# SciLifeLab/TIDDIT

Hardware: AMD Instinct MI355X
Metric: cov bins/sec, 30x WGS synthetic (signals clustered/sec: see 'dbscan') (higher is better)
Workload: dtype int64; 1 GPU; BASELINE configs[1]: coverage histogram, 24 contigs x 125000000 bp (3.00 Gb), 30x 150-bp sorted stream, 500-bp bins, q>=20 filter; contigs split over the 1 rank(s); reads=600000000, bins=6000000

## Files before the change

tiddit_amd/csrc/tdt_coverage.hip:

```cpp
extern const char *const tdt_variant_coverage;
const char *const tdt_variant_coverage = ""
#ifdef COV_MIN_WAVES
    " COV_MIN_WAVES"
#endif
#ifdef COV_MIN_WAVES1
    " COV_MIN_WAVES1"
#endif
#ifdef COV_MIN_WAVES1_4
    " COV_MIN_WAVES1_4"
#endif
#ifdef COV_MIN_WAVES4
    " COV_MIN_WAVES4"
#endif
#ifdef COV_RPL
    " COV_RPL"
#endif
#ifdef COV_RPL1
    " COV_RPL1"
#endif
#ifdef COV_SPARES1
    " COV_SPARES1"
#endif
#ifdef COV_WIN
    " COV_WIN"
#endif
#ifdef COV_WIN1
    " COV_WIN1"
#endif
    ;

#include "tdt_common.h"

#include <algorithm>
#include <thread>

#define COV_THREADS 256
#ifndef COV_RPL
#define COV_RPL 8
#endif
#ifndef COV_RPL1
#define COV_RPL1 4
#endif
#define COV_READS_PER_BLOCK 16384
#ifndef COV_WIN
#define COV_WIN 2048
#endif
#define COV_LUT_LDS_MAX 1024
#define COV_PUSH_CHUNK (4u << 20)
#define COV_STATUS_BYTES (128 + COV_KEPT_SLOTS * 128)
#define COV_KEPT_SLOTS 512

struct CovItem {
    const int32_t *start;
    const int32_t *end;
    const uint8_t *mapq;
    const uint16_t *flag;
    const unsigned long long *packed;
    unsigned long long n;
    unsigned long long *acc;
    const unsigned long long *lut_end;
    int nbins;
    int aligned;
    unsigned first_block;
    unsigned binned;
};

struct CovParams {
    CovItem it;
    const CovItem *items;
    int n_items;
    int bin_size;
    unsigned magic;
    int shift;
    int min_q;
    int margin;
    unsigned xmax, m15;
    int k15;
    const unsigned long long *lut_main;
    unsigned long long one;
    int *status;
    unsigned long long *kept;
};

__device__ __forceinline__ int cov_div(int x, unsigned magic, int shift) {
    return shift < 0 ? x : (int)(__umulhi((unsigned)x, magic) >> shift);
}

#define DPP_WAVE_SHL1 0x130
#define DPP_WAVE_SHR1 0x138

template <int CTRL>
__device__ __forceinline__ unsigned long long dpp_u64(unsigned long long v) {
    const unsigned lo = __builtin_amdgcn_update_dpp(0u, (unsigned)v, CTRL, 0xf, 0xf, true);
    const unsigned hi = __builtin_amdgcn_update_dpp(0u, (unsigned)(v >> 32), CTRL, 0xf, 0xf, true);
    return ((unsigned long long)hi << 32) | lo;
}

#define COV_DPP_SHR1 "row_shr:1 row_mask:0xf bank_mask:0xf bound_ctrl:0"
#define COV_DPP_SHR2 "row_shr:2 row_mask:0xf bank_mask:0xf bound_ctrl:0"
#define COV_DPP_SHR4 "row_shr:4 row_mask:0xf bank_mask:0xf bound_ctrl:0"
#define COV_DPP_SHR8 "row_shr:8 row_mask:0xf bank_mask:0xf bound_ctrl:0"
#define COV_DPP_BC15 "row_bcast:15 row_mask:0xa bank_mask:0xf"
#define COV_DPP_BC31 "row_bcast:31 row_mask:0xc bank_mask:0xf"
#define COV_SCAN_ALL(STEP) \
    "s_nop 1\n\t" STEP(COV_DPP_SHR1) STEP(COV_DPP_SHR2) STEP(COV_DPP_SHR4) STEP(COV_DPP_SHR8) STEP(COV_DPP_BC15) STEP(COV_DPP_BC31) "s_nop 1"
#define COV_SCAN_STEP(CTRL)                                                                     \
    "v_add_co_u32_dpp %0, vcc, %0, %0 " CTRL "\n\t"                                             \
    "v_addc_co_u32_dpp %1, vcc, %1, %1, vcc " CTRL "\n\t"                                       \
    "v_add_co_u32_dpp %2, vcc, %2, %2 " CTRL "\n\t"                                             \
    "v_addc_co_u32_dpp %3, vcc, %3, %3, vcc " CTRL "\n\t"                                       \
    "v_add_co_u32_dpp %4, vcc, %4, %4 " CTRL "\n\t"                                             \
    "v_addc_co_u32_dpp %5, vcc, %5, %5, vcc " CTRL "\n\t"

__device__ __forceinline__ void wave_scan3_u64(unsigned long long &a0, unsigned long long &a1, unsigned long long &a2) {
    unsigned l0 = (unsigned)a0, h0 = (unsigned)(a0 >> 32), l1 = (unsigned)a1, h1 = (unsigned)(a1 >> 32),
             l2 = (unsigned)a2, h2 = (unsigned)(a2 >> 32);
    asm volatile(COV_SCAN_ALL(COV_SCAN_STEP) : "+v"(l0), "+v"(h0), "+v"(l1), "+v"(h1), "+v"(l2), "+v"(h2)::"vcc", "memory");
    a0 = ((unsigned long long)h0 << 32) | l0;
    a1 = ((unsigned long long)h1 << 32) | l1;
    a2 = ((unsigned long long)h2 << 32) | l2;
}

__device__ __forceinline__ unsigned long long cov_mask_lt(unsigned a, unsigned lim_uniform) {
    unsigned long long m;
    asm("v_cmp_gt_u32_e64 %0, %1, %2" : "=s"(m) : "s"(lim_uniform), "v"(a));
    return m;
}
__device__ __forceinline__ unsigned long long cov_mask_eq0(unsigned a) {
    unsigned long long m;
    asm("v_cmp_eq_u32_e64 %0, 0, %1" : "=s"(m) : "v"(a));
    return m;
}
__device__ __forceinline__ unsigned long long cov_mask_ne0(unsigned a) {
    unsigned long long m;
    asm("v_cmp_ne_u32_e64 %0, 0, %1" : "=s"(m) : "v"(a));
// ... 65 lines not shown
}

template <int RPL>
struct CovTile {
    int s[RPL], e[RPL];
    unsigned mq[RPL / 4];
    unsigned fl[RPL / 2];
};

template <int RPL>
__device__ __forceinline__ CovTile<RPL> cov_load(const CovItem &P, unsigned long long idx, unsigned long long r1) {
    CovTile<RPL> t;
    if (P.aligned && idx + RPL <= r1) {
#pragma unroll
        for (int k = 0; k < RPL / 4; k++) {
            const int4 s4 = *reinterpret_cast<const int4 *>(P.start + idx + 4 * k);
            const int4 e4 = *reinterpret_cast<const int4 *>(P.end + idx + 4 * k);
            t.s[4 * k] = s4.x; t.s[4 * k + 1] = s4.y; t.s[4 * k + 2] = s4.z; t.s[4 * k + 3] = s4.w;
            t.e[4 * k] = e4.x; t.e[4 * k + 1] = e4.y; t.e[4 * k + 2] = e4.z; t.e[4 * k + 3] = e4.w;
        }
        if (RPL == 8) {
            const uint2 m2 = *reinterpret_cast<const uint2 *>(P.mapq + idx);
            const uint4 f4 = *reinterpret_cast<const uint4 *>(P.flag + idx);
            t.mq[0] = m2.x; t.mq[RPL / 4 - 1] = m2.y;
            t.fl[0] = f4.x; t.fl[1] = f4.y; t.fl[RPL / 2 - 2] = f4.z; t.fl[RPL / 2 - 1] = f4.w;
        } else {
            t.mq[0] = *reinterpret_cast<const unsigned *>(P.mapq + idx);
            const uint2 f2 = *reinterpret_cast<const uint2 *>(P.flag + idx);
            t.fl[0] = f2.x; t.fl[1] = f2.y;
        }
    } else {
#pragma unroll
        for (int k = 0; k < RPL / 4; k++) t.mq[k] = 0;
#pragma unroll
        for (int k = 0; k < RPL / 2; k++) t.fl[k] = 0;
#pragma unroll
        for (int j = 0; j < RPL; j++) {
            const bool ok = idx + j < r1;
            t.s[j] = ok ? P.start[idx + j] : 0;
            t.e[j] = ok ? P.end[idx + j] : 1;
            t.mq[j / 4] |= (ok ? (unsigned)P.mapq[idx + j] : 0u) << (8 * (j & 3));
            t.fl[j / 2] |= (ok ? (unsigned)P.flag[idx + j] : 0x4u) << (16 * (j & 1));
        }
    }
    return t;
}

template <int RPL>
struct CovTileP {
    unsigned long long w[RPL];
};

template <int RPL>
__device__ __forceinline__ CovTileP<RPL> cov_load_packed(const CovItem &P, unsigned long long idx, unsigned long long r1) {
    CovTileP<RPL> t;
    if (P.aligned && idx + RPL <= r1) {
#pragma unroll
        for (int k = 0; k < RPL / 2; k++) {
            const ulonglong2 v = *reinterpret_cast<const ulonglong2 *>(P.packed + idx + 2 * k);
            t.w[2 * k] = v.x;
            t.w[2 * k + 1] = v.y;
        }
    } else {
#pragma unroll
        for (int j = 0; j < RPL; j++) t.w[j] = idx + j < r1 ? P.packed[idx + j] : (1ull << 62);
    }
    return t;
}

__global__ void cov_pack(const int32_t *__restrict__ start, const int32_t *__restrict__ end, const uint8_t *__restrict__ mapq,
                         const uint16_t *__restrict__ flag, unsigned long long n, unsigned long long *__restrict__ out) {
    unsigned long long i = (unsigned long long)blockIdx.x * blockDim.x + threadIdx.x;
    const unsigned long long stride = (unsigned long long)gridDim.x * blockDim.x;
    for (; i < n; i += stride) out[i] = cov_pack_record(start[i], end[i], mapq[i], flag[i]);
}

__global__ void cov_pack_binned(const int32_t *__restrict__ start, const int32_t *__restrict__ end, const uint8_t *__restrict__ mapq,
                                const uint16_t *__restrict__ flag, unsigned long long n, int nbins, unsigned z, unsigned magic, int shift, int mode1,
                                unsigned long long *__restrict__ out) {
    unsigned long long i = (unsigned long long)blockIdx.x * blockDim.x + threadIdx.x;
    const unsigned long long stride = (unsigned long long)gridDim.x * blockDim.x;
    for (; i < n; i += stride) out[i] = cov_bin_record(start[i], end[i], mapq[i], flag[i], nbins, z, magic, shift, mode1 != 0);
}

#define COV_DBIT 48
#define COV_LOWMASK ((1ull << COV_DBIT) - 1ull)
#ifndef COV_WIN1
#define COV_WIN1 2048
#endif
#define COV_DQMAX 256
#ifndef COV_SPARES1
#define COV_SPARES1 64
#endif

#ifndef COV_MIN_WAVES
#define COV_MIN_WAVES 4
#endif
#ifndef COV_MIN_WAVES4
#define COV_MIN_WAVES4 3
#endif
#ifndef COV_MIN_WAVES1
#define COV_MIN_WAVES1 6
#endif
#ifndef COV_MIN_WAVES1_4
#define COV_MIN_WAVES1_4 4
#endif
template <bool LDS_LUT, int MODE, bool Z1, int RPL, int REC>
__global__ __launch_bounds__(COV_THREADS, MODE == 1 ? (REC ? COV_MIN_WAVES1 : COV_MIN_WAVES1_4) : (REC ? COV_MIN_WAVES : COV_MIN_WAVES4)) void cov_accumulate(CovParams P) {
    constexpr bool PACKED = REC != 0;
    extern __shared__ __attribute__((aligned(16))) unsigned long long smem[];
    constexpr int WIN = MODE == 1 ? COV_WIN1 : COV_WIN;
    constexpr int TILE = COV_THREADS * RPL;
    int *s_wsum = reinterpret_cast<int *>(smem);
    int *s_tbin = s_wsum + 4;
    int *s_rtot = reinterpret_cast<int *>(smem + 12);
    unsigned long long *win = smem + 12 + (MODE == 1 ? 16 : 0);
    unsigned long long *lutS = win + WIN + (MODE == 1 ? COV_SPARES1 : 2);

    const int tid = threadIdx.x;
    const int lane = tid & 63;
    CovItem I = P.it;
    unsigned blk = blockIdx.x;
    if (P.n_items > 0) {
        int lo = 0, hi = P.n_items;
        while (hi - lo > 1) {
            const int mid = (lo + hi) >> 1;
            if (P.items[mid].first_block <= blk) lo = mid;
            else hi = mid;
        }
        I = P.items[lo];
        blk -= I.first_block;
    }
    const unsigned long long r0 = (unsigned long long)blk * COV_READS_PER_BLOCK;
    const unsigned long long r1 = min(I.n, r0 + COV_READS_PER_BLOCK);
    const unsigned z = (unsigned)P.bin_size;
    const int last_bin = I.nbins - 1;
    auto div = [&](int x) { return Z1 ? x : (int)(__umulhi((unsigned)x, P.magic) >> P.shift); };

    auto load_tile = [&](unsigned long long idx) {
        if constexpr (PACKED) return cov_load_packed<RPL>(I, idx, r1);
        else return cov_load<RPL>(I, idx, r1);
    };
    auto cur = load_tile(r0 + (unsigned long long)tid * RPL);

    for (int i = tid; i < WIN + 2; i += COV_THREADS) win[i] = 0;
    if (LDS_LUT) {
        for (unsigned i = tid; i <= z; i += COV_THREADS) {
            const unsigned long long v = P.lut_main[i];
            lutS[i] = v;
            lutS[i + z + 1] = I.lut_end[i];
            if (MODE == 0 && !Z1) {
                unsigned long long *pr = lutS + 2 * (z + 1);
                pr[2 * i] = v;
                pr[2 * i + 1] = 0;
                pr[2 * (z + 1) + 2 * i] = 0;
                pr[2 * (z + 1) + 2 * i + 1] = v;
            }
            if (MODE == 1) {
                unsigned long long *tabA = lutS + 2 * (z + 1), *tabB = tabA + (z + 1), *tabL = tabB + (z + 1);
                tabA[i] = v & 0xffffffffull;
                tabB[i] = v << 32;
                tabL[i] = v - (1ull << COV_DBIT);
                if (i == 0) tabL[z + 1] = 0;
            }
        }
    }
    auto bin_of_read = [&](unsigned long long idx) {
        if constexpr (REC == 2) return (int)((unsigned)I.packed[idx] >> 2);
        int s = PACKED ? (int)(unsigned)I.packed[idx] : I.start[idx];
        s = s < 0 ? 0 : s;
        const int b = div(s);
        return b < I.nbins ? b : I.nbins - 1;
    };
    if (tid < COV_READS_PER_BLOCK / TILE) {
        const unsigned long long tl = min(r0 + (unsigned long long)(tid + 1) * TILE, r1) - 1;
        s_tbin[tid] = bin_of_read(tl);
    }
    int base = bin_of_read(r0);
    __syncthreads();
    auto lut = [&](unsigned i) -> unsigned long long {
        if (LDS_LUT) return lutS[i];
        return i <= z ? P.lut_main[i] : I.lut_end[i - z - 1];
    };

    auto contribute = [&](int bin, unsigned long long v) {
        const unsigned off = (unsigned)(bin - base);
        if (off < (unsigned)WIN) atomicAdd(&win[off], v);
        else if ((unsigned)bin <= (unsigned)last_bin) cov_global_add(I.acc, bin, v);
    };

    auto slow_read = [&](int s, int e) {
        const int fb = div(s);
        const int eb = div(e - 1);
        if (fb == eb) {
            contribute(fb, lut((unsigned)(e - s)));
        } else {
            contribute(fb, lut((unsigned)(fb + 1) * z - (unsigned)s));
            const unsigned bl = (unsigned)(e - 1) - (unsigned)eb * z;
            contribute(eb, lut(eb < last_bin ? bl : bl + z + 1));
            for (int b = fb + 1; b < eb; b++) contribute(b, P.one);
        }
    };

    auto spill = [&]() {
        __syncthreads();
        if constexpr (MODE == 1) {
            constexpr int PER = WIN / COV_THREADS;
            static_assert(PER == 8 && COV_THREADS == 256, "the packed resolve is written for eight rows of 256 words");
            unsigned long long w[PER];
#pragma unroll
            for (int k = 0; k < PER; k++) w[k] = win[k * COV_THREADS + tid];
            int pk[PER / 2];
#pragma unroll
            for (int j = 0; j < PER / 2; j++)
                pk[j] = (int)((long long)w[2 * j] >> COV_DBIT) + (int)((unsigned)((long long)w[2 * j + 1] >> COV_DBIT) << 16);
            wave_scan4_i32(pk[0], pk[1], pk[2], pk[3]);
            int incl[PER];
#pragma unroll
            for (int j = 0; j < PER / 2; j++) {
                incl[2 * j] = (int)(short)(pk[j] & 0xffff);
                incl[2 * j + 1] = (pk[j] - incl[2 * j]) >> 16;
            }
            const int wv = tid >> 6;
            if (lane == 63) {
#pragma unroll
                for (int k = 0; k < PER; k++) s_rtot[k * 4 + wv] = incl[k];
            }
            __syncthreads();
            int tot = lane < 4 * PER ? s_rtot[lane] : 0, z1 = 0, z2 = 0, z3 = 0;
            const int own = tot;
            wave_scan4_i32(tot, z1, z2, z3);
            const int excl = tot - own;
            const unsigned sh = (unsigned)__builtin_ctzll(P.one);
#pragma unroll
            for (int k = 0; k < PER; k++) {
                const int run = incl[k] + __builtin_amdgcn_readlane(excl, k * 4 + wv);
                const unsigned long long v = (w[k] & COV_LOWMASK) + ((unsigned long long)(long long)run << sh);
                const int i = k * COV_THREADS + tid;
                if (w[k]) win[i] = 0;
                if (v) {
                    if (base + i <= last_bin) atomicAdd(&I.acc[base + i], v);
                }
            }
            __syncthreads();
            return;
        }
        for (int i = tid; i < WIN; i += COV_THREADS) {
            const unsigned long long v = win[i];
            if (v) {
                if (base + i <= last_bin) atomicAdd(&I.acc[base + i], v);
                win[i] = 0;
            }
        }
    };

    unsigned nkept = 0;
    unsigned nkept_s = 0;
    bool bad = false;

    for (unsigned long long t0 = r0; t0 < r1; t0 += TILE) {
        auto nxt = cur;
        if (t0 + TILE < r1) nxt = load_tile(t0 + TILE + (unsigned long long)tid * RPL);

        if (t0 != r0) {
            const int step = (int)((t0 - r0) / TILE);
            if (s_tbin[step] + P.margin >= base + WIN) {
                const int nb = s_tbin[step - 1];
                if (nb != base) {
                    spill();
                    __syncthreads();
                    base = nb;
                }
            }
        }

        if constexpr (REC == 2) {
            static_assert(LDS_LUT && !Z1, "binned records exist for 2 <= bin_size < 1024");
            const unsigned K4 = (unsigned)cur.w[0] & ~3u;
            const int K = (int)(K4 >> 2);
            const unsigned ko = (unsigned)(K - base);
            const unsigned minq24 = (unsigned)P.min_q << 24, qlim = (64u - (unsigned)P.min_q) << 24;
            unsigned long long slow_any = 0;
            unsigned long long a0 = 0, a1 = 0, a2 = 0;
            if constexpr (MODE == 0) {
                const bool safe = ko < (unsigned)(WIN - 3);
                const unsigned kw = safe ? ko : 0u;
                const unsigned tA = (unsigned)(size_t)(lutS + 2 * (z + 1)), zb4 = (z + 1u) << 2;
                const unsigned notsafe = safe ? 0u : 8u;
#pragma unroll
                for (int j = 0; j < RPL; j++) {
                    const unsigned lo = (unsigned)cur.w[j], hi = (unsigned)(cur.w[j] >> 32);
                    const unsigned d = lo - K4;
                    const unsigned long long m_cand = cov_mask_lt(hi - minq24, qlim);
                    const unsigned long long m_fast = m_cand & cov_mask_eq0((d & ~5u) | notsafe);
                    nkept_s += (unsigned)__builtin_popcountll(m_fast);
                    slow_any |= m_cand & ~m_fast;
                    const unsigned tab = __umul24(d & 4u, zb4) + tA;
                    const unsigned xa = cov_select(m_fast, (hi & 0x3ff0u) + tab, tA);
                    const ulonglong2 X = cov_lds_read128(xa);
                    const unsigned long long m_multi = m_fast & cov_mask_ne0(d & 1u);
                    const unsigned ya = cov_select(m_multi, (((hi >> 14) & 0x3ffu) << 4) + tab, tA);
                    const ulonglong2 Y = cov_lds_read128(ya);
                    a0 += X.x;
                    a1 += X.y + Y.x;
                    a2 += Y.y;
                }
                if (slow_any) {
                    const unsigned long long idx = t0 + (unsigned long long)tid * RPL;
#pragma unroll
                    for (int j = 0; j < RPL; j++) {
                        unsigned lo = (unsigned)cur.w[j], hi = (unsigned)(cur.w[j] >> 32);
                        asm volatile("" : "+v"(lo), "+v"(hi));
                        const unsigned d = lo - K4;
                        if ((hi - minq24 < qlim) && !(safe & ((d & ~5u) == 0u))) {
                            if ((lo & 3u) == COV_BN_INVALID || idx + j >= r1) bad = true;
                            else { nkept++; slow_read(I.start[idx + j], I.end[idx + j]); }
                        }
                    }
// ... 252 lines not shown
#pragma unroll
                for (int j = 0; j < RPL; j++)
                    if (slowmask & (1u << j)) {
                        const int s = sv[j], e = true_end(j);
                        if (s < 0 || e <= s || div(e - 1) > last_bin) bad = true;
                        else { nkept++; slow_read(s, e); }
                    }
            }
        }
        cur = nxt;
    }

    for (int d = 32; d > 0; d >>= 1) nkept += __shfl_down(nkept, d);
    nkept += nkept_s;
    if (lane == 0 && nkept)
        atomicAdd(P.kept + (size_t)((blockIdx.x * (COV_THREADS / 64) + (tid >> 6)) % COV_KEPT_SLOTS) * 16, (unsigned long long)nkept);
    if (bad) atomicOr(P.status, 1);

    spill();
}

__global__ void cov_finalize(const long long *__restrict__ acc, double *__restrict__ out, long long n, double inv_scale,
                             int *status) {
    long long i = (long long)blockIdx.x * blockDim.x + threadIdx.x;
    const long long stride = (long long)gridDim.x * blockDim.x;
    bool inexact = false;
    for (; i < n; i += stride) {
        const long long a = acc[i];
        if (a >= (1ll << 53) || a < 0) inexact = true;
        out[i] = (double)a * inv_scale;
    }
    if (inexact) atomicOr(status, 2);
}

struct tdt_cov {
    tdt_ctx *ctx = nullptr;
    int n_contigs = 0;
    int bin_size = 0;
    int S = 0;
    bool small_bins = false;
    unsigned xmax = 0, m15 = 0;
    int k15 = 0;
    unsigned magic = 0;
    int shift = 0;
    std::vector<int64_t> len, nbins, off;
    std::vector<int> end_bin_size;
    int64_t total_bins = 0;
    unsigned long long *d_acc = nullptr;
    unsigned long long *d_lut_main = nullptr;
    unsigned long long *d_lut_end = nullptr;
    int *d_status = nullptr;
    unsigned long long *d_kept = nullptr;
    int *d_nbins = nullptr;
    void *d_stage[2] = {nullptr, nullptr};
    void *h_stage[2] = {nullptr, nullptr};
    hipEvent_t slot_ev[2] = {nullptr, nullptr};
    int slot_used[2] = {0, 0};
    int next_slot = 0;
};

static bool build_lut(std::vector<unsigned long long> &lut, int bin_size, int den, int S) {
    const double scale = ldexp(1.0, S);
    for (int b = 0; b <= bin_size; b++) {
        volatile float q = (float)b / (float)den;
        double f = (double)q * scale;
        unsigned long long fx = (unsigned long long)f;
        if ((double)fx != f) return false;
        lut[b] = fx;
    }
    return true;
}

extern "C" int tdt_cov_create(tdt_ctx *ctx, const int64_t *contig_len, int n_contigs, int bin_size, tdt_cov **out) {
    if (!ctx || !contig_len || !out || n_contigs <= 0) {
        tdt_set_error("tdt_cov_create: bad argument");
        return TDT_E_ARG;
    }
    *out = nullptr;
    if (bin_size <= 0 || bin_size > (1 << 24)) {
        tdt_set_error("tdt_cov_create: bin_size %d outside [1, 2^24] (reference: float32 bases are exact only there)",
                      bin_size);
        return TDT_E_ARG;
    }
    TDT_HIP(hipSetDevice(ctx->device));
    tdt_cov *c = new tdt_cov();
    c->ctx = ctx;
    c->n_contigs = n_contigs;
    c->bin_size = bin_size;
    const int L = tdt_ceil_log2_u64((uint64_t)bin_size);
    c->S = 23 + L + 1;
    {
        const char *env = getenv("TIDDIT_COV_MODE");
        const bool can = bin_size >= 2 && c->S <= 31;
        c->small_bins = can;
        if (env && env[0] == '0') c->small_bins = false;
        if (bin_size >= 2 && bin_size + 1 <= COV_LUT_LDS_MAX) {
            c->k15 = 15 + L;
            c->m15 = (unsigned)(((1ull << c->k15) + (unsigned)bin_size - 1) / (unsigned)bin_size);
            const unsigned lim = (unsigned)COV_DQMAX * (unsigned)bin_size;
            c->xmax = lim < 32768u ? lim : 32768u;
            for (unsigned x = 0; x < 32768u; x++)
                if (((x * c->m15) >> c->k15) != x / (unsigned)bin_size) {
                    tdt_set_error("internal: 24-bit division self-check failed for d=%d x=%u", bin_size, x);
                    delete c;
                    return TDT_E_ARG;
                }
// ... 64 lines not shown
        tdt_cov_destroy(c);
        return TDT_E_HIP;
    };
    if ((e = tdt_dev_malloc((void **)&c->d_acc, (size_t)(total > 0 ? total : 1) * 8)) != hipSuccess) return fail("hipMalloc(acc)");
    if ((e = tdt_dev_malloc((void **)&c->d_lut_main, lut_n * 8)) != hipSuccess) return fail("hipMalloc(lut)");
    if ((e = tdt_dev_malloc((void **)&c->d_lut_end, (size_t)n_contigs * lut_n * 8)) != hipSuccess) return fail("hipMalloc(lut_end)");
    if ((e = tdt_dev_malloc((void **)&c->d_status, COV_STATUS_BYTES)) != hipSuccess) return fail("hipMalloc(status)");
    {
        std::vector<int> nb32(c->nbins.begin(), c->nbins.end());
        if ((e = tdt_dev_malloc((void **)&c->d_nbins, (size_t)n_contigs * 4)) != hipSuccess) return fail("hipMalloc(nbins)");
        if ((e = hipMemcpy(c->d_nbins, nb32.data(), (size_t)n_contigs * 4, hipMemcpyHostToDevice)) != hipSuccess) return fail("hipMemcpy(nbins)");
    }
    c->d_kept = (unsigned long long *)((char *)c->d_status + 128);
    if ((e = hipMemcpy(c->d_lut_main, lut.data(), lut_n * 8, hipMemcpyHostToDevice)) != hipSuccess) return fail("hipMemcpy(lut)");
    if ((e = hipMemcpy(c->d_lut_end, lute.data(), (size_t)n_contigs * lut_n * 8, hipMemcpyHostToDevice)) != hipSuccess)
        return fail("hipMemcpy(lut_end)");
    if ((e = hipMemset(c->d_acc, 0, (size_t)(total > 0 ? total : 1) * 8)) != hipSuccess) return fail("hipMemset(acc)");
    if ((e = hipMemset(c->d_status, 0, COV_STATUS_BYTES)) != hipSuccess) return fail("hipMemset(status)");
    for (int i = 0; i < 2; i++)
        if ((e = hipEventCreateWithFlags(&c->slot_ev[i], hipEventDisableTiming)) != hipSuccess) return fail("hipEventCreate");
    *out = c;
    return TDT_OK;
}

extern "C" void tdt_cov_destroy(tdt_cov *c) {
    if (!c) return;
    (void)hipSetDevice(c->ctx->device);
    (void)hipStreamSynchronize(c->ctx->stream);
    if (c->d_acc) (void)hipFree(c->d_acc);
    if (c->d_lut_main) (void)hipFree(c->d_lut_main);
    if (c->d_lut_end) (void)hipFree(c->d_lut_end);
    if (c->d_status) (void)hipFree(c->d_status);
    if (c->d_nbins) (void)hipFree(c->d_nbins);
    for (int i = 0; i < 2; i++) {
        if (c->d_stage[i]) (void)hipFree(c->d_stage[i]);
        if (c->h_stage[i]) (void)hipHostFree(c->h_stage[i]);
        if (c->slot_ev[i]) (void)hipEventDestroy(c->slot_ev[i]);
    }
    delete c;
}

extern "C" int tdt_cov_nbins(tdt_cov *c, int tid, int64_t *nbins, int *end_bin_size) {
    if (!c || tid < 0 || tid >= c->n_contigs) {
        tdt_set_error("tdt_cov_nbins: bad contig id");
        return TDT_E_ARG;
    }
    if (nbins) *nbins = c->nbins[tid];
    if (end_bin_size) *end_bin_size = c->end_bin_size[tid];
    return TDT_OK;
}

extern "C" int tdt_cov_scale_bits(tdt_cov *c) { return c ? c->S : TDT_E_ARG; }

extern "C" int tdt_cov_reset(tdt_cov *c) {
    if (!c) return TDT_E_ARG;
    TDT_HIP(hipSetDevice(c->ctx->device));
    TDT_HIP(hipMemsetAsync(c->d_acc, 0, (size_t)(c->total_bins > 0 ? c->total_bins : 1) * 8, c->ctx->stream));
    TDT_HIP(hipMemsetAsync(c->d_status, 0, COV_STATUS_BYTES, c->ctx->stream));
    return TDT_OK;
}

static CovItem cov_item(tdt_cov *c, int tid, const int32_t *d_start, const int32_t *d_end, const uint8_t *d_mapq,
                        const uint16_t *d_flag, size_t n) {
    CovItem it;
    it.start = d_start;
    it.end = d_end;
    it.mapq = d_mapq;
    it.flag = d_flag;
    it.packed = nullptr;
    it.n = n;
    it.acc = c->d_acc + c->off[tid];
    it.lut_end = c->d_lut_end + (size_t)tid * ((size_t)c->bin_size + 1);
    it.nbins = (int)c->nbins[tid];
    it.aligned = (((uintptr_t)d_start | (uintptr_t)d_end) & 15) == 0 && ((uintptr_t)d_mapq & (COV_RPL - 1)) == 0 &&
                 ((uintptr_t)d_flag & (2 * COV_RPL - 1)) == 0;
    it.first_block = 0;
    it.binned = 0;
    return it;
}

static CovItem cov_item_packed(tdt_cov *c, int tid, const unsigned long long *d_packed, const int32_t *d_end, size_t n) {
    CovItem it = cov_item(c, tid, nullptr, d_end, nullptr, nullptr, n);
    it.packed = d_packed;
    it.aligned = ((uintptr_t)d_packed & 15) == 0;
    return it;
}

static int cov_launch_items(tdt_cov *c, const CovItem &single, const CovItem *d_items, int n_items, unsigned grid, int min_q) {
    CovParams P;
    P.it = single;
    P.items = d_items;
    P.n_items = n_items;
    P.bin_size = c->bin_size;
    P.magic = c->magic;
    P.shift = c->shift;
    P.min_q = min_q;
    P.lut_main = c->d_lut_main;
    P.one = 1ull << c->S;
    P.status = c->d_status;
    P.kept = c->d_kept;
    const bool small = c->small_bins;
    P.margin = small ? COV_DQMAX + 8 : 640 / c->bin_size + 4;
    P.xmax = c->xmax;
    P.m15 = c->m15;
    P.k15 = c->k15;
    const bool lds_lut = c->bin_size + 1 <= COV_LUT_LDS_MAX;
    const size_t lds = 96 + (small ? 128 : 0) + ((size_t)(small ? COV_WIN1 + COV_SPARES1 : COV_WIN + 2)) * 8 + (lds_lut ? 2 * ((size_t)c->bin_size + 1) * 8 : 0) +
                       (small ? (3 * ((size_t)c->bin_size + 1) + 1) * 8 : 0) + ((!small && lds_lut && c->shift >= 0) ? 4 * ((size_t)c->bin_size + 1) * 8 : 0);
    const bool packed = single.packed != nullptr;
    const bool binned = packed && single.binned;
    if (binned && small)
        hipLaunchKernelGGL((cov_accumulate<true, 1, false, COV_RPL1, 2>), dim3(grid), dim3(COV_THREADS), lds, c->ctx->stream, P);
    else if (binned)
        hipLaunchKernelGGL((cov_accumulate<true, 0, false, COV_RPL, 2>), dim3(grid), dim3(COV_THREADS), lds, c->ctx->stream, P);
    else if (small && packed)
        hipLaunchKernelGGL((cov_accumulate<true, 1, false, COV_RPL1, 1>), dim3(grid), dim3(COV_THREADS), lds, c->ctx->stream, P);
    else if (small)
        hipLaunchKernelGGL((cov_accumulate<true, 1, false, COV_RPL1, 0>), dim3(grid), dim3(COV_THREADS), lds, c->ctx->stream, P);
    else if (lds_lut && c->shift >= 0 && packed)
        hipLaunchKernelGGL((cov_accumulate<true, 0, false, COV_RPL, 1>), dim3(grid), dim3(COV_THREADS), lds, c->ctx->stream, P);
    else if (lds_lut && c->shift >= 0)
        hipLaunchKernelGGL((cov_accumulate<true, 0, false, COV_RPL, 0>), dim3(grid), dim3(COV_THREADS), lds, c->ctx->stream, P);
    else if (lds_lut && packed)
        hipLaunchKernelGGL((cov_accumulate<true, 0, true, COV_RPL, 1>), dim3(grid), dim3(COV_THREADS), lds, c->ctx->stream, P);
    else if (lds_lut)
        hipLaunchKernelGGL((cov_accumulate<true, 0, true, COV_RPL, 0>), dim3(grid), dim3(COV_THREADS), lds, c->ctx->stream, P);
    else if (packed)
        hipLaunchKernelGGL((cov_accumulate<false, 0, false, COV_RPL, 1>), dim3(grid), dim3(COV_THREADS), lds, c->ctx->stream, P);
    else
        hipLaunchKernelGGL((cov_accumulate<false, 0, false, COV_RPL, 0>), dim3(grid), dim3(COV_THREADS), lds, c->ctx->stream, P);
    TDT_CHECK_LAUNCH();
    return TDT_OK;
}

static int cov_launch(tdt_cov *c, int tid, const int32_t *d_start, const int32_t *d_end, const uint8_t *d_mapq,
                      const uint16_t *d_flag, size_t n, int min_q) {
    if (n == 0 || c->nbins[tid] == 0) return TDT_OK;
    const unsigned grid = (unsigned)((n + COV_READS_PER_BLOCK - 1) / COV_READS_PER_BLOCK);
    return cov_launch_items(c, cov_item(c, tid, d_start, d_end, d_mapq, d_flag, n), nullptr, 0, grid, min_q);
}

extern "C" int tdt_cov_push_device_multi(tdt_cov *c, int n_items, const int *tids, const int32_t *const *d_start,
                                         const int32_t *const *d_end, const uint8_t *const *d_mapq,
                                         const uint16_t *const *d_flag, const size_t *n, int min_q) {
    if (!c || n_items < 0 || (n_items && (!tids || !d_start || !d_end || !d_mapq || !d_flag || !n))) {
        tdt_set_error("tdt_cov_push_device_multi: bad argument");
        return TDT_E_ARG;
    }
    TDT_HIP(hipSetDevice(c->ctx->device));
    std::vector<CovItem> items;
    unsigned long long blocks = 0;
    for (int i = 0; i < n_items; i++) {
        if (tids[i] < 0 || tids[i] >= c->n_contigs || (n[i] && (!d_start[i] || !d_end[i] || !d_mapq[i] || !d_flag[i]))) {
            tdt_set_error("tdt_cov_push_device_multi: bad item %d", i);
            return TDT_E_ARG;
        }
        if (n[i] == 0 || c->nbins[tids[i]] == 0) continue;
        CovItem it = cov_item(c, tids[i], d_start[i], d_end[i], d_mapq[i], d_flag[i], n[i]);
        it.first_block = (unsigned)blocks;
        blocks += (n[i] + COV_READS_PER_BLOCK - 1) / COV_READS_PER_BLOCK;
        items.push_back(it);
    }
    if (items.empty()) return TDT_OK;
    if (blocks >= 0x7fffffffull) {
        tdt_set_error("tdt_cov_push_device_multi: too many reads for one launch");
        return TDT_E_ARG;
    }
    void *d_items = nullptr;
    int rc = tdt_scratch(c->ctx, 7, items.size() * sizeof(CovItem), &d_items);
    if (rc) return rc;
    TDT_HIP(hipMemcpyAsync(d_items, items.data(), items.size() * sizeof(CovItem), hipMemcpyHostToDevice, c->ctx->stream));
    return cov_launch_items(c, items[0], (const CovItem *)d_items, (int)items.size(), (unsigned)blocks, min_q);
}

extern "C" int tdt_cov_pack_device(tdt_ctx *ctx, const int32_t *d_start, const int32_t *d_end, const uint8_t *d_mapq, const uint16_t *d_flag,
                                   size_t n, uint64_t *d_packed) {
    if (!ctx || (n && (!d_start || !d_end || !d_mapq || !d_flag || !d_packed))) {
        tdt_set_error("tdt_cov_pack_device: bad argument");
        return TDT_E_ARG;
    }
    if (!n) return TDT_OK;
    TDT_HIP(hipSetDevice(ctx->device));
    size_t blocks = (n + 255) / 256;
    if (blocks > 65536) blocks = 65536;
    hipLaunchKernelGGL(cov_pack, dim3((unsigned)blocks), dim3(256), 0, ctx->stream, d_start, d_end, d_mapq, d_flag, (unsigned long long)n,
                       (unsigned long long *)d_packed);
    TDT_CHECK_LAUNCH();
    return TDT_OK;
}

extern "C" int tdt_cov_push_packed_device_multi(tdt_cov *c, int n_items, const int *tids, const uint64_t *const *d_packed,
                                                const int32_t *const *d_end, const size_t *n, int min_q) {
    if (!c || n_items < 0 || (n_items && (!tids || !d_packed || !n))) {
        tdt_set_error("tdt_cov_push_packed_device_multi: bad argument");
        return TDT_E_ARG;
    }
    if (min_q > 63) {
        tdt_set_error("tdt_cov_push_packed_device_multi: packed records keep min(mapq, 63); min_q %d needs the unpacked entry point", min_q);
        return TDT_E_UNSUPPORTED;
    }
    if (min_q < 0) min_q = 0;
    TDT_HIP(hipSetDevice(c->ctx->device));
    std::vector<CovItem> items;
    unsigned long long blocks = 0;
    for (int i = 0; i < n_items; i++) {
        if (tids[i] < 0 || tids[i] >= c->n_contigs || (n[i] && !d_packed[i])) {
            tdt_set_error("tdt_cov_push_packed_device_multi: bad item %d", i);
            return TDT_E_ARG;
        }
        if (n[i] == 0 || c->nbins[tids[i]] == 0) continue;
        CovItem it = cov_item_packed(c, tids[i], (const unsigned long long *)d_packed[i], d_end ? d_end[i] : nullptr, n[i]);
        it.first_block = (unsigned)blocks;
        blocks += (n[i] + COV_READS_PER_BLOCK - 1) / COV_READS_PER_BLOCK;
        items.push_back(it);
    }
    if (items.empty()) return TDT_OK;
    if (blocks >= 0x7fffffffull) {
        tdt_set_error("tdt_cov_push_packed_device_multi: too many reads for one launch");
        return TDT_E_ARG;
    }
    void *d_items = nullptr;
    int rc = tdt_scratch(c->ctx, 7, items.size() * sizeof(CovItem), &d_items);
    if (rc) return rc;
    TDT_HIP(hipMemcpyAsync(d_items, items.data(), items.size() * sizeof(CovItem), hipMemcpyHostToDevice, c->ctx->stream));
    return cov_launch_items(c, items[0], (const CovItem *)d_items, (int)items.size(), (unsigned)blocks, min_q);
}

int tdt_cov_bin_spec(tdt_cov *c, CovBinSpec *out) {
    *out = CovBinSpec();
    if (!c) return TDT_E_ARG;
    if (c->bin_size < 2 || c->bin_size + 1 > COV_LUT_LDS_MAX) return TDT_OK;
    out->z = (unsigned)c->bin_size;
    out->magic = c->magic;
    out->shift = c->shift;
    out->mode1 = c->small_bins ? 1 : 0;
    out->d_nbins = c->d_nbins;
    out->n_contigs = c->n_contigs;
    return TDT_OK;
}

extern "C" int tdt_cov_pack_binned_device(tdt_cov *c, int tid, const int32_t *d_start, const int32_t *d_end, const uint8_t *d_mapq,
                                          const uint16_t *d_flag, size_t n, uint64_t *d_binned) {
    if (!c || tid < 0 || tid >= c->n_contigs || (n && (!d_start || !d_end || !d_mapq || !d_flag || !d_binned))) {
        tdt_set_error("tdt_cov_pack_binned_device: bad argument");
        return TDT_E_ARG;
    }
    CovBinSpec sp;
    tdt_cov_bin_spec(c, &sp);
    if (!sp.z) {
        tdt_set_error("tdt_cov_pack_binned_device: binned records exist for 2 <= bin_size < 1024 (this histogram: %d)", c->bin_size);
        return TDT_E_UNSUPPORTED;
    }
    if (!n) return TDT_OK;
    TDT_HIP(hipSetDevice(c->ctx->device));
    size_t blocks = (n + 255) / 256;
    if (blocks > 65536) blocks = 65536;
    hipLaunchKernelGGL(cov_pack_binned, dim3((unsigned)blocks), dim3(256), 0, c->ctx->stream, d_start, d_end, d_mapq, d_flag, (unsigned long long)n,
                       (int)c->nbins[tid], sp.z, sp.magic, sp.shift, sp.mode1, (unsigned long long *)d_binned);
    TDT_CHECK_LAUNCH();
    return TDT_OK;
}

extern "C" int tdt_cov_push_binned_device_multi(tdt_cov *c, int n_items, const int *tids, const uint64_t *const *d_binned,
                                                const int32_t *const *d_start, const int32_t *const *d_end, const size_t *n, int min_q) {
    if (!c || n_items < 0 || (n_items && (!tids || !d_binned || !d_start || !d_end || !n))) {
        tdt_set_error("tdt_cov_push_binned_device_multi: bad argument");
        return TDT_E_ARG;
    }
    if (c->bin_size < 2 || c->bin_size + 1 > COV_LUT_LDS_MAX) {
        tdt_set_error("tdt_cov_push_binned_device_multi: binned records exist for 2 <= bin_size < 1024 (this histogram: %d)", c->bin_size);
        return TDT_E_UNSUPPORTED;
    }
    if (min_q > 63) {
        tdt_set_error("tdt_cov_push_binned_device_multi: records keep min(mapq, 63); min_q %d needs the unpacked entry point", min_q);
        return TDT_E_UNSUPPORTED;
    }
    if (min_q < 0) min_q = 0;
    TDT_HIP(hipSetDevice(c->ctx->device));
    std::vector<CovItem> items;
    unsigned long long blocks = 0;
    for (int i = 0; i < n_items; i++) {
        if (tids[i] < 0 || tids[i] >= c->n_contigs || (n[i] && (!d_binned[i] || !d_start[i] || !d_end[i]))) {
            tdt_set_error("tdt_cov_push_binned_device_multi: bad item %d (the literal path needs the start and end arrays)", i);
            return TDT_E_ARG;
        }
        if (n[i] == 0 || c->nbins[tids[i]] == 0) continue;
        CovItem it = cov_item_packed(c, tids[i], (const unsigned long long *)d_binned[i], d_end[i], n[i]);
        it.start = d_start[i];
        it.binned = 1;
        it.first_block = (unsigned)blocks;
        blocks += (n[i] + COV_READS_PER_BLOCK - 1) / COV_READS_PER_BLOCK;
        items.push_back(it);
    }
    if (items.empty()) return TDT_OK;
    if (blocks >= 0x7fffffffull) {
        tdt_set_error("tdt_cov_push_binned_device_multi: too many reads for one launch");
        return TDT_E_ARG;
    }
    void *d_items = nullptr;
    int rc = tdt_scratch(c->ctx, 7, items.size() * sizeof(CovItem), &d_items);
    if (rc) return rc;
    TDT_HIP(hipMemcpyAsync(d_items, items.data(), items.size() * sizeof(CovItem), hipMemcpyHostToDevice, c->ctx->stream));
    return cov_launch_items(c, items[0], (const CovItem *)d_items, (int)items.size(), (unsigned)blocks, min_q);
}

extern "C" int tdt_cov_push_device(tdt_cov *c, int tid, const int32_t *d_start, const int32_t *d_end,
                                   const uint8_t *d_mapq, const uint16_t *d_flag, size_t n, int min_q) {
    if (!c || tid < 0 || tid >= c->n_contigs || (n && (!d_start || !d_end || !d_mapq || !d_flag))) {
        tdt_set_error("tdt_cov_push_device: bad argument");
        return TDT_E_ARG;
    }
    TDT_HIP(hipSetDevice(c->ctx->device));
    return cov_launch(c, tid, d_start, d_end, d_mapq, d_flag, n, min_q);
}

extern "C" int tdt_cov_push(tdt_cov *c, int tid, const int32_t *start, const int32_t *end, const uint8_t *mapq,
                            const uint16_t *flag, size_t n, int min_q) {
    if (!c || tid < 0 || tid >= c->n_contigs || (n && (!start || !end || !mapq || !flag))) {
        tdt_set_error("tdt_cov_push: bad argument");
        return TDT_E_ARG;
    }
    TDT_HIP(hipSetDevice(c->ctx->device));
    const size_t chunk = COV_PUSH_CHUNK;
    const size_t slot_bytes = chunk * 12;
    for (size_t o = 0; o < n; o += chunk) {
        const size_t m = n - o < chunk ? n - o : chunk;
        const int s = c->next_slot;
        c->next_slot ^= 1;
        if (!c->h_stage[s]) {
            TDT_HIP(hipHostMalloc(&c->h_stage[s], slot_bytes, hipHostMallocDefault));
            TDT_HIP(tdt_dev_malloc(&c->d_stage[s], slot_bytes));
        }
        if (c->slot_used[s]) TDT_HIP(hipEventSynchronize(c->slot_ev[s]));
        char *h = (char *)c->h_stage[s];
        char *d = (char *)c->d_stage[s];
        const size_t o_end = chunk * 4, o_flag = chunk * 8, o_mapq = chunk * 10;
        if (m >= (1u << 18) && tdt_host_thread_count() >= 4) {
            std::thread t1([&] { memcpy(h, start + o, m * 4); });
            std::thread t2([&] { memcpy(h + o_end, end + o, m * 4); });
            std::thread t3([&] { memcpy(h + o_flag, flag + o, m * 2); });
            memcpy(h + o_mapq, mapq + o, m);
            t1.join();
            t2.join();
            t3.join();
        } else {
            memcpy(h, start + o, m * 4);
            memcpy(h + o_end, end + o, m * 4);
            memcpy(h + o_flag, flag + o, m * 2);
            memcpy(h + o_mapq, mapq + o, m);
        }
        if (m == chunk) {
            TDT_HIP(hipMemcpyAsync(d, h, chunk * 11, hipMemcpyHostToDevice, c->ctx->stream));
        } else {
            TDT_HIP(hipMemcpyAsync(d, h, m * 4, hipMemcpyHostToDevice, c->ctx->stream));
            TDT_HIP(hipMemcpyAsync(d + o_end, h + o_end, m * 4, hipMemcpyHostToDevice, c->ctx->stream));
            TDT_HIP(hipMemcpyAsync(d + o_flag, h + o_flag, m * 2, hipMemcpyHostToDevice, c->ctx->stream));
// ... 119 lines not shown
```

Baseline: 6.513 billion bins/s.

## Make coverage kernel persistent, walking contiguous chunks with cross-chunk window carry

The accumulate kernel now launches only as many blocks as can be resident (queried by occupancy). Each block walks a contiguous range of 16K-read chunks, keeping its LDS window and LUT across chunks and prefetching the next chunk's first tile. This cuts per-block setup, repeated LUT and window initialisation and boundary spills. Item descriptors with at most 32 entries now travel inline as kernel arguments instead of needing an H2D copy, and reset uses a custom zeroing kernel instead of two memsets. The cost is more complex carry and spill logic across chunk and contig boundaries, plus load imbalance when chunks differ in cost.

```diff
diff --git a/tiddit_amd/csrc/tdt_coverage.hip b/tiddit_amd/csrc/tdt_coverage.hip
--- a/tiddit_amd/csrc/tdt_coverage.hip
+++ b/tiddit_amd/csrc/tdt_coverage.hip
@@ -27,6 +27,9 @@
 #ifdef COV_WIN1
     " COV_WIN1"
 #endif
+#ifdef COV_WALK
+    " COV_WALK"
+#endif
     ;
 
 #include "tdt_common.h"
@@ -49,6 +52,7 @@
 #define COV_PUSH_CHUNK (4u << 20)
 #define COV_STATUS_BYTES (128 + COV_KEPT_SLOTS * 128)
 #define COV_KEPT_SLOTS 512
+#define COV_LDS_HEAD 20
 
 struct CovItem {
     const int32_t *start;
@@ -65,10 +69,13 @@
     unsigned binned;
 };
 
+#define COV_ITEMS_KERNARG 32
+
 struct CovParams {
     CovItem it;
     const CovItem *items;
     int n_items;
+    unsigned chunk_q, chunk_r;
     int bin_size;
     unsigned magic;
     int shift;
@@ -80,7 +87,26 @@
     unsigned long long one;
     int *status;
     unsigned long long *kept;
+    CovItem inl[COV_ITEMS_KERNARG];
 };
+static_assert(sizeof(CovParams) <= 3072, "CovParams travels as kernel arguments");
+
+#ifndef COV_WALK
+#define COV_WALK 15
+#endif
+
+__device__ __forceinline__ CovItem cov_item_load(const CovItem *p) {
+#if defined(__HIP_DEVICE_COMPILE__)
+    typedef const unsigned long long __attribute__((address_space(4))) *cov_c64;
+    const cov_c64 w = reinterpret_cast<cov_c64>(reinterpret_cast<size_t>(p));
+    union { unsigned long long u[sizeof(CovItem) / 8]; CovItem it; } x;
+#pragma unroll
+    for (unsigned k = 0; k < sizeof(CovItem) / 8; k++) x.u[k] = w[k];
+    return x.it;
+#else
+    return *p;
+#endif
+}
 
 __device__ __forceinline__ int cov_div(int x, unsigned magic, int shift) {
     return shift < 0 ? x : (int)(__umulhi((unsigned)x, magic) >> shift);
@@ -252,19 +278,27 @@
 };
 
 template <int RPL>
-__device__ __forceinline__ CovTileP<RPL> cov_load_packed(const CovItem &P, unsigned long long idx, unsigned long long r1) {
+__device__ __forceinline__ CovTileP<RPL> cov_load_packed(const CovItem &P, unsigned long long t0, unsigned long long r1, unsigned lane_off) {
     CovTileP<RPL> t;
-    if (P.aligned && idx + RPL <= r1) {
+#if defined(__HIP_DEVICE_COMPILE__)
+    typedef const unsigned long long __attribute__((address_space(1))) *cov_g64;
+    typedef unsigned long long cov_g2u64 __attribute__((ext_vector_type(2)));
+    const cov_g64 base = reinterpret_cast<cov_g64>(reinterpret_cast<size_t>(P.packed + t0));
+    const unsigned cnt = (unsigned)min(r1 - t0, (unsigned long long)COV_READS_PER_BLOCK);
+    if (P.aligned && lane_off + RPL <= cnt) {
 #pragma unroll
         for (int k = 0; k < RPL / 2; k++) {
-            const ulonglong2 v = *reinterpret_cast<const ulonglong2 *>(P.packed + idx + 2 * k);
+            const cov_g2u64 v = *reinterpret_cast<const cov_g2u64 __attribute__((address_space(1))) *>(base + lane_off + 2 * k);
             t.w[2 * k] = v.x;
             t.w[2 * k + 1] = v.y;
         }
     } else {
 #pragma unroll
-        for (int j = 0; j < RPL; j++) t.w[j] = idx + j < r1 ? P.packed[idx + j] : (1ull << 62);
-    }
+        for (int j = 0; j < RPL; j++) t.w[j] = lane_off + j < cnt ? base[lane_off + j] : (1ull << 62);
+    }
+#else
+    (void)P; (void)t0; (void)r1; (void)lane_off;
+#endif
     return t;
 }
 
@@ -312,36 +346,42 @@
     constexpr int WIN = MODE == 1 ? COV_WIN1 : COV_WIN;
     constexpr int TILE = COV_THREADS * RPL;
     int *s_wsum = reinterpret_cast<int *>(smem);
+    constexpr int NT = COV_READS_PER_BLOCK / TILE;
     int *s_tbin = s_wsum + 4;
-    int *s_rtot = reinterpret_cast<int *>(smem + 12);
-    unsigned long long *win = smem + 12 + (MODE == 1 ? 16 : 0);
+    int *s_rtot = reinterpret_cast<int *>(smem + COV_LDS_HEAD);
+    unsigned long long *win = smem + COV_LDS_HEAD + (MODE == 1 ? 16 : 0);
     unsigned long long *lutS = win + WIN + (MODE == 1 ? COV_SPARES1 : 2);
 
     const int tid = threadIdx.x;
     const int lane = tid & 63;
+    unsigned c = blockIdx.x * P.chunk_q + min(blockIdx.x, P.chunk_r);
+    const unsigned c1 = c + P.chunk_q + (blockIdx.x < P.chunk_r ? 1u : 0u);
+    auto item_at = [&](int i) -> CovItem { return P.items ? cov_item_load(P.items + i) : P.inl[i]; };
     CovItem I = P.it;
-    unsigned blk = blockIdx.x;
+    unsigned blk = c;
+    int it_idx = 0;
     if (P.n_items > 0) {
         int lo = 0, hi = P.n_items;
         while (hi - lo > 1) {
             const int mid = (lo + hi) >> 1;
-            if (P.items[mid].first_block <= blk) lo = mid;
+            if (item_at(mid).first_block <= blk) lo = mid;
             else hi = mid;
         }
-        I = P.items[lo];
+        I = item_at(lo);
+        it_idx = lo;
         blk -= I.first_block;
     }
-    const unsigned long long r0 = (unsigned long long)blk * COV_READS_PER_BLOCK;
-    const unsigned long long r1 = min(I.n, r0 + COV_READS_PER_BLOCK);
+    unsigned long long r0 = (unsigned long long)blk * COV_READS_PER_BLOCK;
+    unsigned long long r1 = min(I.n, r0 + COV_READS_PER_BLOCK);
     const unsigned z = (unsigned)P.bin_size;
-    const int last_bin = I.nbins - 1;
+    int last_bin = I.nbins - 1;
     auto div = [&](int x) { return Z1 ? x : (int)(__umulhi((unsigned)x, P.magic) >> P.shift); };
 
-    auto load_tile = [&](unsigned long long idx) {
-        if constexpr (PACKED) return cov_load_packed<RPL>(I, idx, r1);
-        else return cov_load<RPL>(I, idx, r1);
+    auto load_tile = [&](const CovItem &it, unsigned long long tile0, unsigned long long end) {
+        if constexpr (PACKED) return cov_load_packed<RPL>(it, tile0, end, (unsigned)tid * RPL);
+        else return cov_load<RPL>(it, tile0 + (unsigned long long)tid * RPL, end);
     };
-    auto cur = load_tile(r0 + (unsigned long long)tid * RPL);
+    auto cur = load_tile(I, r0, r1);
 
     for (int i = tid; i < WIN + 2; i += COV_THREADS) win[i] = 0;
     if (LDS_LUT) {
@@ -365,18 +405,19 @@
             }
         }
     }
-    auto bin_of_read = [&](unsigned long long idx) {
-        if constexpr (REC == 2) return (int)((unsigned)I.packed[idx] >> 2);
-        int s = PACKED ? (int)(unsigned)I.packed[idx] : I.start[idx];
+    auto bin_of_read = [&](const CovItem &it, unsigned long long idx) {
+        if constexpr (REC == 2) return (int)((unsigned)it.packed[idx] >> 2);
+        int s = PACKED ? (int)(unsigned)it.packed[idx] : it.start[idx];
         s = s < 0 ? 0 : s;
         const int b = div(s);
-        return b < I.nbins ? b : I.nbins - 1;
+        return b < it.nbins ? b : it.nbins - 1;
     };
-    if (tid < COV_READS_PER_BLOCK / TILE) {
-        const unsigned long long tl = min(r0 + (unsigned long long)(tid + 1) * TILE, r1) - 1;
-        s_tbin[tid] = bin_of_read(tl);
-    }
-    int base = bin_of_read(r0);
+    auto tile_last_bin = [&](const CovItem &it, unsigned long long b0, unsigned long long b1) {
+        return bin_of_read(it, min(b0 + (unsigned long long)(tid + 1) * TILE, b1) - 1);
+    };
+    if (tid < NT) s_tbin[tid] = tile_last_bin(I, r0, r1);
+    unsigned half = 0;
+    int base = bin_of_read(I, r0);
     __syncthreads();
     auto lut = [&](unsigned i) -> unsigned long long {
         if (LDS_LUT) return lutS[i];
@@ -458,12 +499,51 @@
     unsigned nkept_s = 0;
     bool bad = false;
 
-    for (unsigned long long t0 = r0; t0 < r1; t0 += TILE) {
+    for (unsigned long long t0 = r0;; t0 += TILE) {
+        if (t0 >= r1) {
+            if (++c == c1) break;
+            const bool same = (unsigned long long)(blk + 1) * COV_READS_PER_BLOCK < I.n;
+            const int carry = s_tbin[half * 16 + (int)((r1 - r0 - 1) / TILE)];
+            if (MODE == 1 || !same) spill();
+            if (same) {
+                blk++;
+            } else {
+                I = item_at(++it_idx);
+                blk = 0;
+                last_bin = I.nbins - 1;
+                if (LDS_LUT)
+                    for (unsigned i = tid; i <= z; i += COV_THREADS) lutS[i + z + 1] = I.lut_end[i];
+            }
+            r0 = (unsigned long long)blk * COV_READS_PER_BLOCK;
+            r1 = min(I.n, r0 + COV_READS_PER_BLOCK);
+            t0 = r0;
+            if (tid < NT) s_tbin[(half ^ 1u) * 16 + tid] = tile_last_bin(I, r0, r1);
+            __syncthreads();
+            half ^= 1u;
+            if (!same) base = bin_of_read(I, r0);
+            else if (MODE == 1) base = carry;
+            else if (s_tbin[half * 16] + P.margin >= base + WIN && carry != base) {
+                spill();
+                __syncthreads();
+                base = carry;
+            }
+        }
         auto nxt = cur;
-        if (t0 + TILE < r1) nxt = load_tile(t0 + TILE + (unsigned long long)tid * RPL);
+        {
+            CovItem In = I;
+            unsigned long long n0 = t0 + TILE, n1 = r1;
+            const bool last_tile = n0 >= r1;
+            if (last_tile && c + 1 < c1) {
+                const bool same = (unsigned long long)(blk + 1) * COV_READS_PER_BLOCK < I.n;
+                if (!same) In = item_at(it_idx + 1);
+                n0 = same ? r0 + COV_READS_PER_BLOCK : 0ull;
+                n1 = min(In.n, n0 + COV_READS_PER_BLOCK);
+            }
+            if (n0 < n1) nxt = load_tile(In, n0, n1);
+        }
 
         if (t0 != r0) {
-            const int step = (int)((t0 - r0) / TILE);
+            const int step = (int)((t0 - r0) / TILE) + (int)half * 16;
             if (s_tbin[step] + P.margin >= base + WIN) {
                 const int nb = s_tbin[step - 1];
                 if (nb != base) {
@@ -822,6 +902,7 @@
     int *d_status = nullptr;
     unsigned long long *d_kept = nullptr;
     int *d_nbins = nullptr;
+    int resident[10] = {0};
     void *d_stage[2] = {nullptr, nullptr};
     void *h_stage[2] = {nullptr, nullptr};
     hipEvent_t slot_ev[2] = {nullptr, nullptr};
@@ -992,11 +1073,23 @@
 
 extern "C" int tdt_cov_scale_bits(tdt_cov *c) { return c ? c->S : TDT_E_ARG; }
 
+__global__ void cov_reset(ulonglong2 *__restrict__ acc, size_t n_acc, ulonglong2 *__restrict__ status, size_t n_status) {
+    const size_t stride = (size_t)gridDim.x * blockDim.x;
+    const ulonglong2 zero = make_ulonglong2(0, 0);
+    for (size_t i = (size_t)blockIdx.x * blockDim.x + threadIdx.x; i < n_acc + n_status; i += stride) {
+        if (i < n_acc) acc[i] = zero;
+        else status[i - n_acc] = zero;
+    }
+}
+
 extern "C" int tdt_cov_reset(tdt_cov *c) {
     if (!c) return TDT_E_ARG;
     TDT_HIP(hipSetDevice(c->ctx->device));
-    TDT_HIP(hipMemsetAsync(c->d_acc, 0, (size_t)(c->total_bins > 0 ? c->total_bins : 1) * 8, c->ctx->stream));
-    TDT_HIP(hipMemsetAsync(c->d_status, 0, COV_STATUS_BYTES, c->ctx->stream));
+    const size_t n_acc = (size_t)c->total_bins / 2, n_status = COV_STATUS_BYTES / 16;
+    size_t blocks = (n_acc + n_status + 255) / 256;
+    if (blocks > 4096) blocks = 4096;
+    hipLaunchKernelGGL(cov_reset, dim3((unsigned)blocks), dim3(256), 0, c->ctx->stream, (ulonglong2 *)c->d_acc, n_acc, (ulonglong2 *)c->d_status, n_status);
+    TDT_CHECK_LAUNCH();
     return TDT_OK;
 }
 
@@ -1026,11 +1119,40 @@
     return it;
 }
 
-static int cov_launch_items(tdt_cov *c, const CovItem &single, const CovItem *d_items, int n_items, unsigned grid, int min_q) {
+template <bool LDS_LUT, int MODE, bool Z1, int RPL, int REC>
+static int cov_launch_one(tdt_cov *c, CovParams &P, unsigned chunks, size_t lds, int slot) {
+    constexpr unsigned walk_bit = REC == 2 ? (MODE == 1 ? 2u : 1u) : REC == 1 ? 4u : 8u;
+    unsigned grid = chunks;
+    if ((COV_WALK) & walk_bit) {
+        if (!c->resident[slot]) {
+            int nb = 0;
+            TDT_HIP(hipOccupancyMaxActiveBlocksPerMultiprocessor(&nb, cov_accumulate<LDS_LUT, MODE, Z1, RPL, REC>, COV_THREADS, lds));
+            c->resident[slot] = nb > 0 ? nb : 1;
+        }
+        const unsigned long long held = (unsigned long long)(c->ctx->num_cu > 0 ? c->ctx->num_cu : 1) * (unsigned)c->resident[slot];
+        if (held < grid) grid = (unsigned)held;
+    }
+    P.chunk_q = chunks / grid;
+    P.chunk_r = chunks % grid;
+    hipLaunchKernelGGL((cov_accumulate<LDS_LUT, MODE, Z1, RPL, REC>), dim3(grid), dim3(COV_THREADS), lds, c->ctx->stream, P);
+    TDT_CHECK_LAUNCH();
+    return TDT_OK;
+}
+
+static int cov_launch_items(tdt_cov *c, const CovItem &single, const CovItem *items, int n_items, unsigned chunks, int min_q) {
     CovParams P;
     P.it = single;
-    P.items = d_items;
+    P.items = nullptr;
     P.n_items = n_items;
+    if (n_items > COV_ITEMS_KERNARG) {
+        void *d_items = nullptr;
+        int rc = tdt_scratch(c->ctx, 7, (size_t)n_items * sizeof(CovItem), &d_items);
+        if (rc) return rc;
+        TDT_HIP(hipMemcpyAsync(d_items, items, (size_t)n_items * sizeof(CovItem), hipMemcpyHostToDevice, c->ctx->stream));
+        P.items = (const CovItem *)d_items;
+    } else if (n_items > 0) {
+        memcpy(P.inl, items, (size_t)n_items * sizeof(CovItem));
+    }
     P.bin_size = c->bin_size;
     P.magic = c->magic;
     P.shift = c->shift;
@@ -1045,32 +1167,20 @@
     P.m15 = c->m15;
     P.k15 = c->k15;
     const bool lds_lut = c->bin_size + 1 <= COV_LUT_LDS_MAX;
-    const size_t lds = 96 + (small ? 128 : 0) + ((size_t)(small ? COV_WIN1 + COV_SPARES1 : COV_WIN + 2)) * 8 + (lds_lut ? 2 * ((size_t)c->bin_size + 1) * 8 : 0) +
+    const size_t lds = COV_LDS_HEAD * 8 + (small ? 128 : 0) + ((size_t)(small ? COV_WIN1 + COV_SPARES1 : COV_WIN + 2)) * 8 + (lds_lut ? 2 * ((size_t)c->bin_size + 1) * 8 : 0) +
                        (small ? (3 * ((size_t)c->bin_size + 1) + 1) * 8 : 0) + ((!small && lds_lut && c->shift >= 0) ? 4 * ((size_t)c->bin_size + 1) * 8 : 0);
     const bool packed = single.packed != nullptr;
     const bool binned = packed && single.binned;
-    if (binned && small)
-        hipLaunchKernelGGL((cov_accumulate<true, 1, false, COV_RPL1, 2>), dim3(grid), dim3(COV_THREADS), lds, c->ctx->stream, P);
-    else if (binned)
-        hipLaunchKernelGGL((cov_accumulate<true, 0, false, COV_RPL, 2>), dim3(grid), dim3(COV_THREADS), lds, c->ctx->stream, P);
-    else if (small && packed)
-        hipLaunchKernelGGL((cov_accumulate<true, 1, false, COV_RPL1, 1>), dim3(grid), dim3(COV_THREADS), lds, c->ctx->stream, P);
-    else if (small)
-        hipLaunchKernelGGL((cov_accumulate<true, 1, false, COV_RPL1, 0>), dim3(grid), dim3(COV_THREADS), lds, c->ctx->stream, P);
-    else if (lds_lut && c->shift >= 0 && packed)
-        hipLaunchKernelGGL((cov_accumulate<true, 0, false, COV_RPL, 1>), dim3(grid), dim3(COV_THREADS), lds, c->ctx->stream, P);
-    else if (lds_lut && c->shift >= 0)
-        hipLaunchKernelGGL((cov_accumulate<true, 0, false, COV_RPL, 0>), dim3(grid), dim3(COV_THREADS), lds, c->ctx->stream, P);
-    else if (lds_lut && packed)
-        hipLaunchKernelGGL((cov_accumulate<true, 0, true, COV_RPL, 1>), dim3(grid), dim3(COV_THREADS), lds, c->ctx->stream, P);
-    else if (lds_lut)
-        hipLaunchKernelGGL((cov_accumulate<true, 0, true, COV_RPL, 0>), dim3(grid), dim3(COV_THREADS), lds, c->ctx->stream, P);
-    else if (packed)
-        hipLaunchKernelGGL((cov_accumulate<false, 0, false, COV_RPL, 1>), dim3(grid), dim3(COV_THREADS), lds, c->ctx->stream, P);
-    else
-        hipLaunchKernelGGL((cov_accumulate<false, 0, false, COV_RPL, 0>), dim3(grid), dim3(COV_THREADS), lds, c->ctx->stream, P);
-    TDT_CHECK_LAUNCH();
-    return TDT_OK;
+    if (binned && small) return cov_launch_one<true, 1, false, COV_RPL1, 2>(c, P, chunks, lds, 0);
+    if (binned) return cov_launch_one<true, 0, false, COV_RPL, 2>(c, P, chunks, lds, 1);
+    if (small && packed) return cov_launch_one<true, 1, false, COV_RPL1, 1>(c, P, chunks, lds, 2);
+    if (small) return cov_launch_one<true, 1, false, COV_RPL1, 0>(c, P, chunks, lds, 3);
+    if (lds_lut && c->shift >= 0 && packed) return cov_launch_one<true, 0, false, COV_RPL, 1>(c, P, chunks, lds, 4);
+    if (lds_lut && c->shift >= 0) return cov_launch_one<true, 0, false, COV_RPL, 0>(c, P, chunks, lds, 5);
+    if (lds_lut && packed) return cov_launch_one<true, 0, true, COV_RPL, 1>(c, P, chunks, lds, 6);
+    if (lds_lut) return cov_launch_one<true, 0, true, COV_RPL, 0>(c, P, chunks, lds, 7);
+    if (packed) return cov_launch_one<false, 0, false, COV_RPL, 1>(c, P, chunks, lds, 8);
+    return cov_launch_one<false, 0, false, COV_RPL, 0>(c, P, chunks, lds, 9);
 }
 
 static int cov_launch(tdt_cov *c, int tid, const int32_t *d_start, const int32_t *d_end, const uint8_t *d_mapq,
@@ -1106,11 +1216,7 @@
         tdt_set_error("tdt_cov_push_device_multi: too many reads for one launch");
         return TDT_E_ARG;
     }
-    void *d_items = nullptr;
-    int rc = tdt_scratch(c->ctx, 7, items.size() * sizeof(CovItem), &d_items);
-    if (rc) return rc;
-    TDT_HIP(hipMemcpyAsync(d_items, items.data(), items.size() * sizeof(CovItem), hipMemcpyHostToDevice, c->ctx->stream));
-    return cov_launch_items(c, items[0], (const CovItem *)d_items, (int)items.size(), (unsigned)blocks, min_q);
+    return cov_launch_items(c, items[0], items.data(), (int)items.size(), (unsigned)blocks, min_q);
 }
 
 extern "C" int tdt_cov_pack_device(tdt_ctx *ctx, const int32_t *d_start, const int32_t *d_end, const uint8_t *d_mapq, const uint16_t *d_flag,
@@ -1159,11 +1265,7 @@
         tdt_set_error("tdt_cov_push_packed_device_multi: too many reads for one launch");
         return TDT_E_ARG;
     }
-    void *d_items = nullptr;
-    int rc = tdt_scratch(c->ctx, 7, items.size() * sizeof(CovItem), &d_items);
-    if (rc) return rc;
-    TDT_HIP(hipMemcpyAsync(d_items, items.data(), items.size() * sizeof(CovItem), hipMemcpyHostToDevice, c->ctx->stream));
-    return cov_launch_items(c, items[0], (const CovItem *)d_items, (int)items.size(), (unsigned)blocks, min_q);
+    return cov_launch_items(c, items[0], items.data(), (int)items.size(), (unsigned)blocks, min_q);
 }
 
 int tdt_cov_bin_spec(tdt_cov *c, CovBinSpec *out) {
@@ -1237,11 +1339,7 @@
         tdt_set_error("tdt_cov_push_binned_device_multi: too many reads for one launch");
         return TDT_E_ARG;
     }
-    void *d_items = nullptr;
-    int rc = tdt_scratch(c->ctx, 7, items.size() * sizeof(CovItem), &d_items);
-    if (rc) return rc;
-    TDT_HIP(hipMemcpyAsync(d_items, items.data(), items.size() * sizeof(CovItem), hipMemcpyHostToDevice, c->ctx->stream));
-    return cov_launch_items(c, items[0], (const CovItem *)d_items, (int)items.size(), (unsigned)blocks, min_q);
+    return cov_launch_items(c, items[0], items.data(), (int)items.size(), (unsigned)blocks, min_q);
 }
 
 extern "C" int tdt_cov_push_device(tdt_cov *c, int tid, const int32_t *d_start, const int32_t *d_end,
```

Result: no change. 6.462 billion bins/s (-0.8%).
